# btourn/Neural-Networks-parallel-training-with-MPI

Measured on AMD Instinct MI355X. Metric: samples_per_sec_whole_node, higher is better.
Workload: dtype bf16; 1 GPU; model=mlp_512x4_regression(512-512-512-512-1), global_batch=8192, parallelism=dp1, rows_per_gpu=8192, uneven_split=False, device=cuda, comm=none, graph=True, graph_chunk=128, overlap=True, grouped=True, schedule=rowband, grad_wire_bytes_per_rank=0, n_buckets=3

## Files before the change

neural-networks-parallel-training-with-mpi_amd/csrc/bindings.cpp:

```cpp
#include <pybind11/pybind11.h>
#include <pybind11/stl.h>

#include <stdexcept>
#include <string>

#include "comm/rccl_comm.h"
#include "host/shm_comm.h"
#include "kernels/common.h"
#include "kernels/kernels.h"
#include "knobs.h"

namespace py = pybind11;
using namespace nnmpi;

namespace nnmpi {
void set_sgd_tiles(int v);
}
#if NNMPI_EXPERIMENTS_BUILD
namespace nnmpi {
void set_wgrad_multi_stamps(unsigned long long* buf);
void set_wgm_tile(int t);
}
#endif

// ... 43 lines not shown
  pk.n = (int)py::len(l);
  for (int t = 0; t < pk.n; ++t) {
    auto e = l[t].cast<py::tuple>();
    pk.start[t] = e[0].cast<long long>();
    pk.M[t] = e[1].cast<int>();
    pk.N[t] = e[2].cast<int>();
    pk.pkf[t] = P<bf16>(e[3].cast<uptr>());
    pk.pkd[t] = P<bf16>(e[4].cast<uptr>());
  }
  return true;
}

static void rb_packed_args(const py::object& o, RowbandArgs& a) {
  if (o.is_none()) return;
  auto l = o.cast<py::list>();
  if ((int)py::len(l) != a.nh) throw std::runtime_error("rowband: one (Pf, Pd) pair per hidden layer");
  for (int i = 0; i < a.nh; ++i) {
    auto t = l[i].cast<py::tuple>();
    a.Pf[i] = P<const bf16>(t[0].cast<uptr>());
    a.Pd[i] = P<const bf16>(t[1].cast<uptr>());
  }
}

PYBIND11_MODULE(_nnmpi_hip, m) {
  m.doc() = "MI355X-native kernels and RCCL runtime for nnmpi_amd";

  m.def("arch", []() {
    int dev = 0;
    check(hipGetDevice(&dev), "hipGetDevice");
    hipDeviceProp_t prop;
    check(hipGetDeviceProperties(&prop, dev), "hipGetDeviceProperties");
    return std::string(prop.gcnArchName);
  });
  m.def("cu_count", []() {
    int dev = 0, n = 0;
    check(hipGetDevice(&dev), "hipGetDevice");
    check(hipDeviceGetAttribute(&n, hipDeviceAttributeMultiprocessorCount, dev), "attr");
    return n;
  });
  m.def("source_hash", []() { return std::string(nnmpi_source_hash()); });
  m.def("rccl_version", []() {
    int v = 0;
    ncclGetVersion(&v);
    return v;
  });

  m.def("linear_fwd_bf16", [](uptr X, int ldx, uptr W, int ldw, uptr bias, uptr Y, int ldy, int M,
                              int N, int K, int act, uptr s) {
    check(linear_fwd_bf16(P<const bf16>(X), ldx, P<const bf16>(W), ldw, P<const float>(bias),
                          P<bf16>(Y), ldy, M, N, K, act, S(s)), "linear_fwd_bf16");
  });
  m.def("linear_dgrad_bf16", [](uptr dZ, int lddz, uptr W, int ldw, uptr Ap, int ldap, uptr dX,
                                int lddx, int M, int N, int K, int act, uptr s) {
    check(linear_dgrad_bf16(P<const bf16>(dZ), lddz, P<const bf16>(W), ldw, P<const bf16>(Ap), ldap,
                            P<bf16>(dX), lddx, M, N, K, act, S(s)), "linear_dgrad_bf16");
  });
  m.def("gemm_w4_fwd", [](uptr X, int ldx, uptr W, int ldw, uptr bias, uptr Y, int ldy, int M, int N,
                          int K, int act, uptr s) {
    if (!gemm_w4_fwd) throw std::runtime_error("gemm_w4_fwd: experiments build only (NNMPI_BUILD_EXPERIMENTS=1)");
    check(gemm_w4_fwd(P<const bf16>(X), ldx, P<const bf16>(W), ldw, P<const float>(bias), P<bf16>(Y),
                      ldy, M, N, K, act, S(s)), "gemm_w4_fwd");
  });
  m.def("set_gemm_impl", knob(&set_gemm_impl));
  m.def("get_gemm_impl", &get_gemm_impl);
  m.def("set_gemm_tile", knob(&set_gemm_tile));
  m.def("set_gemm_variant", knob(&set_gemm_variant));
  m.def("set_fwd_variant", knob(&set_fwd_variant));
  m.def("set_store_policy", knob(&set_store_policy));
  m.def("set_slab_store_policy", knob(&set_slab_store_policy));
  m.def("set_pp256_order", knob(&set_pp256_order));
  m.def("set_head_xcd_rows", knob(&set_head_xcd_rows));
  m.def("linear_fwd_bf16_stamped", [](uptr X, int ldx, uptr W, int ldw, uptr bias, uptr Y, int ldy,
                                      int M, int N, int K, uptr st, uptr s) {
#if NNMPI_EXPERIMENTS_BUILD
    check(linear_fwd_bf16_stamped(P<const bf16>(X), ldx, P<const bf16>(W), ldw, P<const float>(bias),
                                  P<bf16>(Y), ldy, M, N, K, P<unsigned long long>(st), S(s)),
          "linear_fwd_bf16_stamped");
#else
    experiments_only("linear_fwd_bf16_stamped");
#endif
  });
  m.def("set_group_async", knob(&set_group_async));
  m.def("set_wgrad_splits", knob(&set_wgrad_splits));
  m.def("wgrad_workspace_bytes", &wgrad_workspace_bytes);
  m.def("wgrad_splits", &wgrad_splits);
  m.def("linear_wgrad_bf16", [](uptr dZ, int lddz, uptr X, int ldx, uptr dW, uptr db, int M, int N,
                                int K, uptr ws, uptr s, py::object sgd) {
    SgdFuse f{};
    const bool fu = to_sgd(sgd, f);
    check(linear_wgrad_bf16(P<const bf16>(dZ), lddz, P<const bf16>(X), ldx, P<float>(dW), P<float>(db),
                            M, N, K, P<float>(ws), S(s), fu ? &f : nullptr), "linear_wgrad_bf16");
  }, py::arg("dZ"), py::arg("lddz"), py::arg("X"), py::arg("ldx"), py::arg("dW"), py::arg("db"),
     py::arg("M"), py::arg("N"), py::arg("K"), py::arg("ws"), py::arg("s"), py::arg("sgd") = py::none());
  m.def("wide_pair_wgrad_ok", &wide_pair_wgrad_ok);
  m.def("wide_pair_dgrad_ok", &wide_pair_dgrad_ok);
  m.def("set_wide_pair", knob(&set_wide_pair));
  m.def("experiments_built", &experiments_built);
  m.def("experiments_on", &experiments_on);
  m.def("cu_hold", [](int blocks, double seconds, uptr s) {
    if (!cu_hold) throw std::runtime_error("cu_hold: experiments build only (NNMPI_BUILD_EXPERIMENTS=1)");
    check(cu_hold(blocks, seconds, S(s)), "cu_hold");
  });
  m.def("set_head_general_valu", knob(&set_head_general_valu));
  m.def("head_general_mfma_ok", &head_general_mfma_ok);
  m.def("set_sgd_epilogue", knob(&set_sgd_epilogue));
  m.def("set_pp_prefetch", knob(&set_pp_prefetch));
  m.def("set_rb_band_map", knob(&set_rb_band_map));
  m.def("cu_mask_stream", [](std::vector<uint32_t> mask) {
    if (!exp_cu_mask_stream)
      throw std::runtime_error("cu_mask_stream: experiments build only (NNMPI_BUILD_EXPERIMENTS=1)");
    hipStream_t st = nullptr;
    check(exp_cu_mask_stream(mask.data(), (int)mask.size(), &st), "cu_mask_stream");
    return reinterpret_cast<uptr>(st);
  });
  m.def("stream_destroy", [](uptr st) { check(hipStreamDestroy(S(st)), "stream_destroy"); });
  m.def("set_stage_epi", knob(&set_stage_epi));
  m.def("wgrad_defer_ok", &wgrad_defer_ok);
  m.def("linear_wgrad_bf16_out16_defer", [](uptr dZ, int lddz, uptr X, int ldx, uptr dW16, uptr db16,
                                            int M, int N, int K, py::object other, uptr g16o, uptr s) {
    SgdFuse f{};
    if (!to_sgd(other, f)) throw std::runtime_error("deferred update needs its SGD operands");
    check(linear_wgrad_bf16_out16_defer(P<const bf16>(dZ), lddz, P<const bf16>(X), ldx, P<bf16>(dW16),
                                        P<bf16>(db16), M, N, K, f, P<const bf16>(g16o), S(s)),
          "linear_wgrad_bf16_out16_defer");
  });
  m.def("wide_pair_wgrad_dgrad_bf16", [](uptr dZ, int lddz, uptr X, int ldx, uptr dW, uptr db, int M,
                                         int N, int K, py::object sgd, uptr dZ2, int lddz2, uptr W2,
                                         int ldw2, uptr Ap2, int ldap2, uptr dX2, int lddx2, int M2,
                                         int N2, int K2, int act2, uptr s) {
    WgradArgs w{P<const bf16>(dZ), lddz, P<const bf16>(X), ldx, P<float>(dW), P<float>(db), M, N, K,
                nullptr, SgdFuse{}};
    to_sgd(sgd, w.sg);
    DgradArgs d{P<const bf16>(dZ2), lddz2, P<const bf16>(W2), ldw2, P<const bf16>(Ap2), ldap2,
                P<bf16>(dX2), lddx2, M2, N2, K2, act2};
    check(wide_pair(w, &d, nullptr, S(s)), "wide_pair_wgrad_dgrad_bf16");
  });
  m.def("wide_pair_wgrad_wgrad_bf16", [](uptr dZ, int lddz, uptr X, int ldx, uptr dW, uptr db, int M,
                                         int N, int K, py::object sgd, uptr dZ2, int lddz2, uptr X2,
                                         int ldx2, uptr dW2, uptr db2, int M2, int N2, int K2,
                                         py::object sgd2, uptr s) {
    WgradArgs w{P<const bf16>(dZ), lddz, P<const bf16>(X), ldx, P<float>(dW), P<float>(db), M, N, K,
                nullptr, SgdFuse{}};
    to_sgd(sgd, w.sg);
    WgradArgs w2{P<const bf16>(dZ2), lddz2, P<const bf16>(X2), ldx2, P<float>(dW2), P<float>(db2), M2,
                 N2, K2, nullptr, SgdFuse{}};
    to_sgd(sgd2, w2.sg);
    check(wide_pair(w, nullptr, &w2, S(s)), "wide_pair_wgrad_wgrad_bf16");
  });
  m.def("linear_wgrad_bf16_out16", [](uptr dZ, int lddz, uptr X, int ldx, uptr dW16, uptr db16,
                                      int M, int N, int K, uptr s) {
    check(linear_wgrad_bf16_ex(P<const bf16>(dZ), lddz, P<const bf16>(X), ldx, nullptr, nullptr,
                               M, N, K, nullptr, S(s),
                               nullptr, nullptr, P<bf16>(dW16), P<bf16>(db16)),
          "linear_wgrad_bf16_out16");
  });
  m.def("gemm_bf16_tile", [](uptr A, int lda, int la, uptr B, int ldb, int lb, int M, int N, int K,
                             uptr C, int ldc, int tile, uptr s) {
    check(gemm_bf16_generic_tile(P<const bf16>(A), lda, la, P<const bf16>(B), ldb, lb, M, N, K,
                                 P<float>(C), ldc, tile, S(s)), "gemm_bf16_tile");
  });
  m.def("gemm_bf16", [](uptr A, int lda, int la, uptr B, int ldb, int lb, int M, int N, int K, uptr C,
                        int ldc, uptr s) {
    check(gemm_bf16_generic(P<const bf16>(A), lda, la, P<const bf16>(B), ldb, lb, M, N, K, P<float>(C),
                            ldc, S(s)), "gemm_bf16");
  });
  m.def("linear_fwd_f32", [](uptr X, int ldx, uptr W, int ldw, uptr bias, uptr Y, int ldy, int M,
// ... 402 lines not shown
```

neural-networks-parallel-training-with-mpi_amd/csrc/kernels/gemm_bf16.hip:

```cpp
#include "gemm_tiles.h"
#include "knobs.h"

namespace nnmpi {

static int g_stage_epi = -1;
void set_stage_epi(int on) { g_stage_epi = on; }
static int stage_epi() {
  if (g_stage_epi < 0) {
    const char* e = knob_env("NNMPI_STAGE_EPI");
    g_stage_epi = (e && e[0] == '1') ? 1 : 0;
  }
  return g_stage_epi;
}
static int g_sgd_serial = -1;
void set_sgd_epilogue(int form) { g_sgd_serial = form; }
static int sgd_serial() {
  if (g_sgd_serial < 0) {
    const char* e = knob_env("NNMPI_SGD_SERIAL");
    g_sgd_serial = (e && e[0] >= '0' && e[0] <= '2') ? e[0] - '0' : 0;
  }
  return g_sgd_serial;
}
static int g_store_pol = 0;

// ... 1020 lines not shown
  int* flag = reinterpret_cast<int*>(smem + 60 * 1024);
  if (tid == 0) {
    const int old = __hip_atomic_fetch_add(cw, 1, __ATOMIC_RELAXED, __HIP_MEMORY_SCOPE_AGENT);
    int mode = 0;
    if (old == S - 1) {
      mode = 2;
    } else {
      int polls = 0;
      while (ld_sc1_i(cw) < S && ++polls < WGM_SPIN) __builtin_amdgcn_s_sleep(8);
      if (polls < WGM_SPIN &&
          __hip_atomic_fetch_add(cw + 1 + split, 1, __ATOMIC_RELAXED, __HIP_MEMORY_SCOPE_AGENT) == 0)
        mode = 1;
    }
    if (mode == 2)
      mode = __hip_atomic_fetch_add(cw + 1 + split, 1, __ATOMIC_RELAXED, __HIP_MEMORY_SCOPE_AGENT) == 0 ? 2 : 3;
    flag[0] = mode;
  }
  __syncthreads();
  const int mode = flag[0];
  __syncthreads();
  if (mode == 0) return;
  if (mode == 1 || mode == 2) wgm_portion(p, f, smem, tx, ty, split);
  if (mode >= 2) {
    for (int o = 1; o < S; ++o) {
      const int pp = (split + o) % S;
      if (tid == 0)
        flag[0] = __hip_atomic_fetch_add(cw + 1 + pp, 1, __ATOMIC_RELAXED, __HIP_MEMORY_SCOPE_AGENT) == 0;
      __syncthreads();
      const int mine = flag[0];
      __syncthreads();
      if (mine) wgm_portion(p, f, smem, tx, ty, pp);
    }
  }
}

template <int GA, int NS, bool ST = false, bool FIX = false>
__global__ void __launch_bounds__(GRP_THREADS, (NS == 0 || GA >= 3 || FIX || ST) ? 2 : 4) wgrad_multi_kernel(WgradMultiParams g) {
  extern __shared__ __attribute__((aligned(1024))) char smem[];
  if constexpr (FIX) {
    if ((int)blockIdx.x >= g.gemm_blocks) {
      slab_reduce_any(g.tail_ws, g.tail, blockIdx.x - g.gemm_blocks, g.tail_nb_main, g.tail_nb_bias,
                      reinterpret_cast<f32x4*>(smem));
      return;
    }
  }
  if constexpr (ST) {
    if (threadIdx.x == 0) {
      g.stamps[blockIdx.x * 4 + 0] = __builtin_amdgcn_s_memrealtime();
      g.stamps[blockIdx.x * 4 + 2] = __builtin_amdgcn_s_getreg(20 | (31 << 11));
      g.stamps[blockIdx.x * 4 + 3] = __builtin_amdgcn_s_getreg(4 | (31 << 11));
    }
  }
  int bid = blockIdx.x;
#pragma unroll
  for (int j = 0; j < RB_MAXL; ++j) {
    if (j >= g.nj) break;
    if (bid < g.blocks[j]) {
      const int l = xcd_remap(bid, g.blocks[j]);
      if (l >= g.n[j]) break;
      const int split = l / g.tiles[j], t = l % g.tiles[j];
      unsigned long long* kst = ST ? g.stamps + 1024 * 4 + (long long)blockIdx.x * 128 : nullptr;
      if constexpr (FIX) {
        constexpr int MI = GRP_BM / GRP_WGM / 16, NJ = GRP_BN / GRP_WGN / 16;
        f32x4 acc[MI * NJ], accb[MI];
        dma_gemm_tile<GRP_BM, GRP_BN, GRP_WGM, GRP_WGN, XMAJ, XMAJ, EPI_F32, ACT_NONE, true, NS, GA, ST,
                      true>(g.wg[j], smem, t % g.gx[j], t / g.gx[j], split, kst, acc, accb);
        wgm_fixup(g.wg[j], g.fix[j], smem, t % g.gx[j], t / g.gx[j], split, t, acc, accb);
      } else if constexpr (NS == 0) {
        wg_reg_tile(g.wg[j], smem, t % g.gx[j], t / g.gx[j], split);
      } else {
        dma_gemm_tile<GRP_BM, GRP_BN, GRP_WGM, GRP_WGN, XMAJ, XMAJ, EPI_F32, ACT_NONE, true, NS, GA, ST>(
            g.wg[j], smem, t % g.gx[j], t / g.gx[j], split, kst);
      }
      break;
    }
    bid -= g.blocks[j];
  }
  if constexpr (ST) {
    __syncthreads();
    if (threadIdx.x == 0) g.stamps[blockIdx.x * 4 + 1] = __builtin_amdgcn_s_memrealtime();
  }
}

#if NNMPI_EXPERIMENTS_BUILD
constexpr int WGH_BM = 128, WGH_BN = 64, WGH_WGM = 2, WGH_WGN = 2;
constexpr int WGH_THREADS = 64 * WGH_WGM * WGH_WGN;
constexpr int WGH_SMEM = 2 * (WGH_BM + WGH_BN) * GEMM_BK * 2;

template <int GA>
__global__ void __launch_bounds__(WGH_THREADS, 2) wgrad_multi_h_kernel(WgradMultiParams g) {
  extern __shared__ __attribute__((aligned(1024))) char smem[];
  int bid = blockIdx.x;
#pragma unroll
  for (int j = 0; j < RB_MAXL; ++j) {
    if (j >= g.nj) break;
    if (bid < g.blocks[j]) {
      const int l = xcd_remap(bid, g.blocks[j]);
      if (l >= g.n[j]) break;
      const int split = l / g.tiles[j], t = l % g.tiles[j];
      dma_gemm_tile<WGH_BM, WGH_BN, WGH_WGM, WGH_WGN, XMAJ, XMAJ, EPI_F32, ACT_NONE, true, 2, GA>(
          g.wg[j], smem, t % g.gx[j], t / g.gx[j], split);
      break;
    }
    bid -= g.blocks[j];
  }
}

static int g_wgm_tile = -1;
void set_wgm_tile(int t) { g_wgm_tile = t; }
static int wgm_tile() {
  if (g_wgm_tile < 0) {
    const char* e = knob_env("NNMPI_WGM_TILE");
    g_wgm_tile = (e && e[0] == '1') ? 1 : 0;
  }
  return g_wgm_tile;
}
#else
static constexpr int wgm_tile() { return 0; }
#endif

template <int GA, int NS>
static void* wgm_fn(bool fix, bool st) {
#if NNMPI_EXPERIMENTS_BUILD
  if (fix) return st ? (void*)wgrad_multi_kernel<GA, NS, true, true> : (void*)wgrad_multi_kernel<GA, NS, false, true>;
  return st ? (void*)wgrad_multi_kernel<GA, NS, true, false> : (void*)wgrad_multi_kernel<GA, NS, false, false>;
#else
  return (fix || st) ? nullptr : (void*)wgrad_multi_kernel<GA, NS, false, false>;
#endif
}

static hipError_t wgm_launch(const WgradMultiParams& g, int nb, bool fix, hipStream_t s) {
  static const int env_ga = [] {
    const char* e = knob_env("NNMPI_WGM_ASYNC");
    return (e && e[0] >= '0' && e[0] <= '4') ? e[0] - '0' : -1;
  }();
  int ga = g_group_async >= 0 ? std::min(g_group_async, 4) : env_ga >= 0 ? env_ga : WGM_ASYNC_DEFAULT;
  int ns = wgm_stages();
  if (fix && ns == 0) ns = 2;
  if (ga < 2) ga = 2;
  const bool st = g.stamps != nullptr;
  void* f = nullptr;
#if NNMPI_EXPERIMENTS_BUILD
  if (ns == 0) f = st ? (void*)wgrad_multi_kernel<2, 0, true> : (void*)wgrad_multi_kernel<2, 0>;
#else
  if (ns == 0) f = st ? nullptr : (void*)wgrad_multi_kernel<2, 0>;
#endif
  else if (ns == 3) f = ga == 2 ? wgm_fn<2, 3>(fix, st) : ga == 3 ? wgm_fn<3, 3>(fix, st) : wgm_fn<4, 3>(fix, st);
  else if (ns == WGM_NS) f = ga == 2 ? wgm_fn<2, WGM_NS>(fix, st) : ga == 3 ? wgm_fn<3, WGM_NS>(fix, st)
                                                                   : wgm_fn<4, WGM_NS>(fix, st);
  else f = ga == 2 ? wgm_fn<2, 2>(fix, st) : ga == 3 ? wgm_fn<3, 2>(fix, st) : wgm_fn<4, 2>(fix, st);
  if (!f) return hipErrorNotSupported;
  const int smem = (ns == 0 ? 2 : ns) * (GRP_BM + GRP_BN) * GEMM_BK * 2;
  static void* attr_done[64] = {};
  bool seen = false;
  for (void*& a : attr_done) {
    if (a == f) { seen = true; break; }
    if (!a) { a = f; break; }
  }
  if (!seen) (void)hipFuncSetAttribute(f, hipFuncAttributeMaxDynamicSharedMemorySize, smem);
  hipLaunchKernelGGL(reinterpret_cast<void (*)(WgradMultiParams)>(f), dim3(nb), dim3(GRP_THREADS), smem, s, g);
  return hipGetLastError();
}

int wgrad_multi_splits(int nj, int M, int N, int K) {
  const int tiles = ((M + GRP_BM - 1) / GRP_BM) * ((N + GRP_BN - 1) / GRP_BN);
  const int ksteps = (K + GEMM_BK - 1) / GEMM_BK;
  int s = std::max(1, 256 / std::max(1, nj * tiles));
  s = std::min(s, std::max(1, ksteps / 4));
  if (g_wgrad_splits > 0 && g_wgrad_splits < s) s = g_wgrad_splits;
  return s;
}

hipError_t wgrad_multi(const WgradArgs* jobs, int nj, const int* splits, SlabReduce* pending,
                       hipStream_t s) {
  if (nj < 1 || nj > RB_MAXL) return hipErrorInvalidValue;
  WgradMultiParams g{};
  g.nj = nj;
  int nb = 0;
  for (int j = 0; j < nj; ++j) {
    const WgradArgs& a = jobs[j];
    if (wgrad_tile(a.M, a.N) != 128 || a.db == nullptr || a.ws == nullptr || a.dW16 != nullptr)
      return hipErrorInvalidValue;
    const int want = (splits && splits[j] > 0) ? splits[j] : wgrad_multi_splits(nj, a.M, a.N, a.K);
    GemmParams p;
    const int sp = make_wgrad_s(a, p, pending[j], want);
    if (sp == 1) {
      p.C = a.ws; p.c_split_stride = (long long)a.M * a.N; p.sg = SgdFuse{};
      p.bias_grad = a.ws + (size_t)a.M * a.N; p.bg_split_stride = a.M;
      p.c16 = nullptr; p.bg16 = nullptr;
      pending[j] = SlabReduce{a.ws, 1, (long long)a.M * a.N, a.M, a.N, a.dW, a.N,
                              a.ws + (size_t)a.M * a.N, a.M, a.db, nullptr, 0, 0.f, nullptr, a.sg};
    }
    set_extents<XMAJ, XMAJ>(p);
    p.store_pol = slab_store_pol();
    g.wg[j] = p;
#if NNMPI_EXPERIMENTS_BUILD
    const int bn = wgm_tile() == 1 ? WGH_BN : GRP_BN;
#else
    const int bn = GRP_BN;
#endif
    g.gx[j] = (p.N + bn - 1) / bn;
    g.tiles[j] = g.gx[j] * ((p.M + GRP_BM - 1) / GRP_BM);
    g.n[j] = g.tiles[j] * sp;
    g.blocks[j] = (g.n[j] + 7) & ~7;
    nb += g.blocks[j];
  }
#if NNMPI_EXPERIMENTS_BUILD
  if (wgm_tile() == 1) {
    static const int env_ga = [] {
      const char* e = knob_env("NNMPI_WGM_ASYNC");
      return (e && e[0] >= '2' && e[0] <= '4') ? e[0] - '0' : -1;
    }();
    const int ga = env_ga == 3 ? 3 : env_ga == 4 ? 4 : 2;
    void* f = ga == 3 ? (void*)wgrad_multi_h_kernel<3> : ga == 4 ? (void*)wgrad_multi_h_kernel<4>
                                                               : (void*)wgrad_multi_h_kernel<2>;
    static void* attr_done[4] = {};
    bool seen = false;
    for (void*& a : attr_done) {
      if (a == f) { seen = true; break; }
      if (!a) { a = f; break; }
    }
    if (!seen) (void)hipFuncSetAttribute(f, hipFuncAttributeMaxDynamicSharedMemorySize, WGH_SMEM);
    hipLaunchKernelGGL(reinterpret_cast<void (*)(WgradMultiParams)>(f), dim3(nb), dim3(WGH_THREADS),
                       WGH_SMEM, s, g);
    return hipGetLastError();
  }
#endif
  g.stamps = g_wgm_stamps;
  return wgm_launch(g, nb, false, s);
}

#if NNMPI_EXPERIMENTS_BUILD
int wgrad_fix_counters(int M, int N) {
  return ((M + GRP_BM - 1) / GRP_BM) * ((N + GRP_BN - 1) / GRP_BN) * WGM_CW;
}
#endif

#if NNMPI_EXPERIMENTS_BUILD
hipError_t wgrad_multi_fix(const WgradArgs* jobs, int nj, const int* splits, const WgOut* fix,
                           const SlabReduce* tail, hipStream_t s) {
  if (nj < 1 || nj > RB_MAXL) return hipErrorInvalidValue;
  WgradMultiParams g{};
  g.nj = nj;
// ... 395 lines not shown
```

neural-networks-parallel-training-with-mpi_amd/csrc/kernels/gemm_tiles.h:

```cpp
#pragma once
#include "common.h"
#include "kernels.h"

#include <algorithm>
#include <cstdlib>

namespace nnmpi {

enum Layout : int { KMAJ = 0, XMAJ = 1 };

constexpr int GEMM_BK = 64;
constexpr int GEMM_THREADS = 256;

struct GemmParams {
  const bf16* A;
  const bf16* B;
  int lda, ldb;
  int M, N, K;
  int k_per_split;
  void* C;
  int ldc;
  long long c_split_stride;
  const float* bias;
  const bf16* aux;
// ... 745 lines not shown
      asm volatile("s_waitcnt lgkmcnt(0)" ::: "memory");
      __builtin_amdgcn_sched_barrier(0);
#pragma unroll
      for (int kk = 0; kk < BK / 32; ++kk) {
#pragma unroll
        for (int i = 0; i < MI; ++i)
#pragma unroll
          for (int j = 0; j < NJ; ++j)
            acc[i][j] = __builtin_amdgcn_mfma_f32_16x16x32_bf16(bfr[j][kk], af[i][kk], acc[i][j], 0, 0, 0);
        if constexpr (BIASGRAD) {
          if (do_bg) {
#pragma unroll
            for (int i = 0; i < MI; ++i)
              accb[i] = __builtin_amdgcn_mfma_f32_16x16x32_bf16(ones, af[i][kk], accb[i], 0, 0, 0);
          }
        }
      }
    } else {
#pragma unroll
      for (int kk = 0; kk < BK / 32; ++kk) {
        bf16x8 af[MI], bfr[NJ];
#pragma unroll
        for (int i = 0; i < MI; ++i) af[i] = read_frag<BM, LA>(cur, wm * WM + i * 16, kk, lane);
#pragma unroll
        for (int j = 0; j < NJ; ++j) bfr[j] = read_frag<BN, LB>(cur + A_BYTES, wn * WN + j * 16, kk, lane);
#pragma unroll
        for (int i = 0; i < MI; ++i)
#pragma unroll
          for (int j = 0; j < NJ; ++j)
            acc[i][j] = __builtin_amdgcn_mfma_f32_16x16x32_bf16(bfr[j], af[i], acc[i][j], 0, 0, 0);
        if constexpr (BIASGRAD) {
          if (do_bg) {
#pragma unroll
            for (int i = 0; i < MI; ++i)
              accb[i] = __builtin_amdgcn_mfma_f32_16x16x32_bf16(ones, af[i], accb[i], 0, 0, 0);
          }
        }
      }
    }
    if constexpr (KST) {
      if (tid == 0 && t < 32) kst[4 * t + 3] = __builtin_amdgcn_s_memtime();
    }
    asm volatile("s_waitcnt lgkmcnt(0)" ::: "memory");
  }
  if constexpr (RET) {
#pragma unroll
    for (int i = 0; i < MI; ++i) {
#pragma unroll
      for (int j = 0; j < NJ; ++j) acc_out[i * NJ + j] = acc[i][j];
      accb_out[i] = accb[i];
    }
    return;
  }
  if constexpr (BM == 128 && BN == 128 && NS * STAGE >= 128 * 128 * 4) {
    if (lepi_ok<EPI>(p)) {
      lds_epilogue<WGM, WGN, EPI, ACT>(p, acc, smem, m0, n0, wm, wn, w, lane, split);
      if constexpr (BIASGRAD) {
        if (do_bg && (lane >> 4) == 0) {
#pragma unroll
          for (int i = 0; i < MI; ++i) {
            const int m = m0 + wm * WM + i * 16 + (lane & 15);
            if (m >= p.M) continue;
            float* g = p.bias_grad + split * p.bg_split_stride + m;
            if (p.sg.g_base) sgd_fused_store(p.sg, g, accb[i][0]);
            else *g = accb[i][0];
          }
        }
      }
      return;
    }
  }
  gemm_epilogue<BM, BN, WGM, WGN, EPI, ACT, BIASGRAD>(p, acc, accb, do_bg, m0, n0, wm, wn, lane, split,
                                                      EPI == EPI_BIAS_ACT ? bias_pre : nullptr);
}

template <int BM, int BN, int WGM, int WGN, int LA, int LB, int EPI, int ACT, bool BIASGRAD, int NS>
__global__ void __launch_bounds__(64 * WGM * WGN) gemm_bf16_dma_kernel(GemmParams p) {
  extern __shared__ __attribute__((aligned(1024))) char smem[];
  const int gx = gridDim.x, gy = gridDim.y;
  const int bid = xcd_remap(blockIdx.y * gx + blockIdx.x, gx * gy);
  dma_gemm_tile<BM, BN, WGM, WGN, LA, LB, EPI, ACT, BIASGRAD, NS>(p, smem, bid % gx, bid / gx, blockIdx.z);
}

constexpr int PP_HALF = 16384;
constexpr int PP_BUF = 4 * PP_HALF;
constexpr int PP_SMEM = 2 * PP_BUF;
constexpr int PP_THREADS = 512;

template <bool OTHER = false>
__device__ __forceinline__ void sgd_epilogue_lds_256(const GemmParams& p, const f32x4 (&acc)[8][4],
                                                     char* smem, int m0, int n0, int wm, int wn,
                                                     int w, int lane, int split) {
  const SgdFuse& f = OTHER ? p.sg2 : p.sg;
  const float lr = f.hp[0], mom = f.hp[1], damp = f.hp[2], wd = f.hp[3], gs = f.hp[4];
  const bool nest = f.nesterov != 0, first = f.first != 0;
  const float* cbase = reinterpret_cast<const float*>(p.C) + split * p.c_split_stride;
  const long long base = OTHER ? 0 : cbase - f.g_base;
  f32x4* img = reinterpret_cast<f32x4*>(smem);
#pragma unroll
  for (int h = 0; h < 2; ++h) {
    __syncthreads();
#pragma unroll
    for (int ii = 0; ii < 4; ++ii) {
      const int r = wm * 64 + ii * 16 + (lane & 15);
#pragma unroll
      for (int j = 0; j < 4; ++j) {
        const int cv = ((j >> 1) * 128 + wn * 32 + (j & 1) * 16) / 4 + (lane >> 4);
        img[r * 64 + (cv ^ (r & 15))] = acc[h * 4 + ii][j];
      }
    }
    __syncthreads();
#pragma unroll
    for (int sb = 0; sb < 2; ++sb) {
      f32x4 pv[8], bv[8];
      f32x4 gov[OTHER ? 8 : 1];
#pragma unroll
      for (int k = 0; k < 8; ++k) {
        const int r = w * 16 + sb * 8 + k;
        const long long o = base + (long long)(m0 + h * 128 + r) * p.ldc + n0 + lane * 4;
        pv[k] = *reinterpret_cast<const f32x4*>(f.p_base + o);
        bv[k] = *reinterpret_cast<const f32x4*>(f.m_base + o);
        if constexpr (OTHER) {
          const bf16x4 gq = *reinterpret_cast<const bf16x4*>(p.g16o + o);
          gov[k] = f32x4{(float)gq[0], (float)gq[1], (float)gq[2], (float)gq[3]};
        }
      }
#pragma unroll
      for (int k = 0; k < 8; ++k) {
        const int r = w * 16 + sb * 8 + k;
        const long long o = base + (long long)(m0 + h * 128 + r) * p.ldc + n0 + lane * 4;
        const f32x4 a = img[r * 64 + (lane ^ (r & 15))];
        f32x4 g = a;
        if constexpr (OTHER) {
          g = gov[k];
          bf16x4 o16;
#pragma unroll
          for (int e = 0; e < 4; ++e) o16[e] = (bf16)a[e];
          *reinterpret_cast<bf16x4*>(p.c16 + (long long)(m0 + h * 128 + r) * p.ldc + n0 + lane * 4) = o16;
        }
        f32x4 q = pv[k], b = bv[k];
#pragma unroll
        for (int e = 0; e < 4; ++e) {
          float bb = b[e];
          q[e] = sgd_elem(q[e], g[e], bb, lr, mom, damp, wd, gs, nest, first);
          b[e] = bb;
        }
        *reinterpret_cast<f32x4*>(f.p_base + o) = q;
        if (mom != 0.f) *reinterpret_cast<f32x4*>(f.m_base + o) = b;
        if (f.s_base) {
          bf16x4 sv;
#pragma unroll
          for (int e = 0; e < 4; ++e) sv[e] = (bf16)q[e];
          *reinterpret_cast<bf16x4*>(f.s_base + o) = sv;
        }
      }
    }
  }
}

template <int ACT>
__device__ __forceinline__ void bias_act_lds_256(const GemmParams& p, const f32x4 (&acc)[8][4],
                                                 char* smem, int m0, int n0, int wm, int wn, int w,
                                                 int lane) {
  bf16x4* img = reinterpret_cast<bf16x4*>(smem);
  f32x4 bias[4];
#pragma unroll
// ... 273 lines not shown
```

neural-networks-parallel-training-with-mpi_amd/csrc/kernels/kernels.h:

```cpp
#pragma once
#include "knobs.h"
#include <hip/hip_runtime.h>
#include <stddef.h>
#include <stdint.h>

namespace nnmpi {

typedef __bf16 bf16;

constexpr int RB_MAXL_PK = 4;

struct SgdFuse {
  const float* g_base;
  float* p_base;
  float* m_base;
  bf16* s_base;
  const float* hp;
  int nesterov;
  int first;
};

struct SlabReduce {
  const float* ws;
  int S;
  long long stride;
  int M, N;
  float* out;
  int ldo;
  const float* bws;
  long long bstride;
  float* bout;
  const float* loss_part;
  int n_loss_part;
  float loss_scale;
  float* loss_out;
  SgdFuse sg;
  int sgd_serial = 0;
  bf16* pkf = nullptr;
  bf16* pkd = nullptr;
};

enum Epi : int { EPI_BIAS_ACT = 0, EPI_DACT = 1, EPI_F32 = 2 };
enum Loss : int { LOSS_MSE = 0, LOSS_XENT = 1 };

hipError_t linear_fwd_bf16(const bf16* X, int ldx, const bf16* W, int ldw, const float* bias,
                           bf16* Y, int ldy, int M, int N, int K, int act, hipStream_t s);
__attribute__((weak)) hipError_t gemm_w4_fwd(const bf16* X, int ldx, const bf16* W, int ldw, const float* bias, bf16* Y,
                       int ldy, int M, int N, int K, int act, hipStream_t s);
hipError_t linear_dgrad_bf16(const bf16* dZ, int lddz, const bf16* W, int ldw, const bf16* Aprev,
                             int lda_prev, bf16* dX, int lddx, int M, int N, int K, int act,
                             hipStream_t s);
int wgrad_splits(int M, int N, int K);
void set_gemm_impl(int impl);
int get_gemm_impl();
void set_gemm_tile(int t);
void set_gemm_variant(int v);
void set_fwd_variant(int v);
void set_pp_prefetch(int v);
void set_pp256_order(int epi, int idx);
void set_store_policy(int p);
void set_slab_store_policy(int p);
void set_head_xcd_rows(int v);
hipError_t linear_fwd_bf16_stamped(const bf16* X, int ldx, const bf16* W, int ldw, const float* bias,
                                   bf16* Y, int ldy, int M, int N, int K, unsigned long long* stamps,
                                   hipStream_t s);
void set_group_async(int m);
void set_wgrad_splits(int s);
size_t wgrad_workspace_bytes(int M, int N, int K);
hipError_t linear_wgrad_bf16(const bf16* dZ, int lddz, const bf16* X, int ldx, float* dW,
                             float* db, int M, int N, int K, float* ws, hipStream_t s,
                             const SgdFuse* sgd = nullptr);
hipError_t gemm_bf16_generic(const bf16* A, int lda, int la, const bf16* B, int ldb, int lb,
                             int M, int N, int K, float* C, int ldc, hipStream_t s);
hipError_t gemm_bf16_generic_tile(const bf16* A, int lda, int la, const bf16* B, int ldb, int lb,
                                  int M, int N, int K, float* C, int ldc, int tile, hipStream_t s);
hipError_t splitk_reduce(const float* ws, int S, long long stride, int M, int N, float* out,
                         int ldo, const float* bws, long long bstride, float* bout,
                         const float* loss_part, int n_loss_part, float loss_scale,
                         float* loss_out, hipStream_t s, const SgdFuse* sgd = nullptr);
hipError_t slab_reduce(const SlabReduce& r, hipStream_t s);
hipError_t linear_wgrad_bf16_ex(const bf16* dZ, int lddz, const bf16* X, int ldx, float* dW,
                                float* db, int M, int N, int K, float* ws, hipStream_t s,
                                const SgdFuse* sgd, SlabReduce* pending, bf16* dW16, bf16* db16);
hipError_t linear_wgrad_bf16_deferred(const bf16* dZ, int lddz, const bf16* X, int ldx, float* dW,
                                      float* db, int M, int N, int K, float* ws, hipStream_t s,
                                      const SgdFuse* sgd, SlabReduce* pending);
struct DgradArgs {
  const bf16* dZ; int lddz; const bf16* W; int ldw; const bf16* Aprev; int lda_prev;
  bf16* dX; int lddx; int M, N, K, act;
};
struct WgradArgs {
  const bf16* dZ; int lddz; const bf16* X; int ldx; float* dW; float* db; int M, N, K;
  float* ws; SgdFuse sg;
  bf16* dW16 = nullptr; bf16* db16 = nullptr;
};
void set_bwd_group(int on);
bool bwd_group_supported(int rows, int out_f, int in_f);
hipError_t bwd_group(const DgradArgs* dg, const WgradArgs* wg, const SlabReduce* red,
                     SlabReduce* wg_pending, hipStream_t s);
bool wide_pair_wgrad_ok(int rows, int out_f, int in_f);
bool wide_pair_dgrad_ok(int rows, int out_f, int in_f);
hipError_t wide_pair(const WgradArgs& w1, const DgradArgs* dg, const WgradArgs* w2, hipStream_t s);
void set_wide_pair(int on);
bool experiments_built();
void set_sgd_epilogue(int form);
void set_stage_epi(int on);
bool wgrad_defer_ok(int M, int N, int K);
hipError_t linear_wgrad_bf16_out16_defer(const bf16* dZ, int lddz, const bf16* X, int ldx, bf16* dW16,
                                         bf16* db16, int M, int N, int K, const SgdFuse& other,
                                         const bf16* g16o, hipStream_t s);

constexpr int RB_MAXL = 4;
struct RowbandArgs {
  const bf16* X; int ldx;
  int rows, H, nh, act;
  int in;
  const bf16* Pf[RB_MAXL];
  const bf16* Pd[RB_MAXL];
  const bf16* W[RB_MAXL];
  const float* b[RB_MAXL];
  bf16* a[RB_MAXL];
  bf16* dz[RB_MAXL];
  const float* wh; const float* bh;
  const float* y;
  float inv_count;
  float* wslab; float* bslab; float* loss_part;
  int band_map;
  unsigned long long* stamps = nullptr;
  int out_pol = 0;
  int* zero_words = nullptr;
  int n_zero = 0;
  int* xsync = nullptr;
  float* hx = nullptr;
  int rbs_bands = 0;
  int rbs_map = 0;
  int rbs_local = 0;
  bf16* ka[RB_MAXL] = {};
  bf16* kz[RB_MAXL] = {};
  int kbands = 0;
};
bool rowband_split_ok(int rows, int H, int in, int nh, int act);
void set_rb_split(int v);
void set_rb_wgsmall(int v);
int rowband_error_word();
int rowband_split_stamp_slots();
void set_rb_store_policy(int pol);
void set_rb_fixup(int on);
void set_rowband_stamps(unsigned long long* buf);
int rowband_stamp_slots();
int rowband_blocks(int rows);
// ... 142 lines not shown
```

neural-networks-parallel-training-with-mpi_amd/utils/knobs.py:

```python
from __future__ import annotations

import os
from typing import Dict, Optional

EXPERIMENTS = "NNMPI_EXPERIMENTS"

KNOBS = {
    "NNMPI_ROWBAND": "row-band step schedule (0 off)",
    "NNMPI_ROWBAND_MIN_ROWS": "smallest batch that takes the row-band step",
    "NNMPI_RB_SPLITS": "row-band weight-gradient split-K slabs",
    "NNMPI_RB_PLAN": "row-band split-K plan (0 one launch, 1 phased; RowbandStep::plan)",
    "NNMPI_DEFER": "deferred bucket updates in weight-gradient epilogues (0 off)",
    "NNMPI_DEFER_WAIT": "deferred update waits per chunk / per layer",
    "NNMPI_CHUNK_MIN_TILES": "tiles per output-row chunk bucket",
    "NNMPI_BF16_REDUCE": "bf16 all-reduce algorithm (acc32 | rccl)",
    "NNMPI_F32_REDUCE": "fp32 all-reduce algorithm (ordered | rccl)",
    "NNMPI_SHM": "shared-memory all-reduce of CPU ranks (0: gloo)",
    "NNMPI_CPU_NATIVE": "native host step of tiny CPU models (0: PyTorch)",
    "NNMPI_STAGE_EPI": "LDS-staged 256x256 forward epilogue",
    "NNMPI_SGD_SERIAL": "SGD epilogue form",
    "NNMPI_PP_PREFETCH": "SGD-operand prefetch in the 256x256 weight gradient",
    "NNMPI_RB_BANDMAP": "XCD-contiguous band order of the row-band kernel",
    "NNMPI_RB_STORE": "row-band copy-out store policy (0 plain, 1 nt, 2 sc1)",
    "NNMPI_RB_SPLIT": "column-split row-band kernel for small batches: 0 off, 2 / 4 / 8 blocks per band, else auto",
    "NNMPI_RB_SPLIT_WAVES": "column-split row-band kernel: waves per block at 4 / 2 blocks per band (4 or 8)",
    "NNMPI_RB_WGSMALL": "small-batch row-band weight gradients: 1 un-split tiles with the update fused, 0 split-K slabs",
    "NNMPI_WGS_ASYNC": "small-batch weight-gradient LDS read mode (2 / 3 / 4, dma_gemm_tile ASYNC_TR)",
    "NNMPI_WGS_STAGES": "small-batch weight-gradient DMA ring stages (2 / 3 / 4 / 6 / 8)",
    "NNMPI_RB_FIXUP": "row-band split-K combine inside the weight-gradient launch (0: own launch)",
    "NNMPI_GEMM": "GEMM main loop (1 register-staged, 2 LDS-DMA)",
    "NNMPI_SLAB_STORE": "split-K slab store policy",
    "NNMPI_GROUP": "grouped backward launch (0 off)",
    "NNMPI_GRAPH_UPLOAD": "hipGraphUpload after instantiation (0 off)",
    "NNMPI_PAIR": "wide backward pair launches (experiments build)",
    "NNMPI_COMM_STANDIN": "k:gbps -- k CUs held after every bucket collective (standin.hip)",
    "NNMPI_WG_STAGES": "grouped weight-gradient launch DMA ring stages (default 2; 4)",
    "NNMPI_WG_REG": "register-staged operands in the grouped weight-gradient launch (A/B)",
    "NNMPI_WGM_ASYNC": "LDS read mode of the row-band weight-gradient launch (2; 3 pipelined)",
    "NNMPI_WGM_TILE": "row-band weight-gradient tile (0: 128x128, 8 waves; 1: 128x64, 4 waves)",
    "NNMPI_HEAD_BLOCKS": "block cap of the fused multi-output head (default 256)",
    "NNMPI_HEAD_FUSED": "multi-output head + weight gradient in one kernel (0: two launches)",
}

INTERNAL = {"NNMPI_SUPERVISED", "NNMPI_ATTEMPT", "NNMPI_PROGRESS_FILE", "NNMPI_RESULT_FILE",
            "NNMPI_LAUNCHER", "NNMPI_RDZV_KEY"}


def experiments() -> bool:
    return os.environ.get(EXPERIMENTS) == "1"


def knob(name: str, default: Optional[str] = None) -> Optional[str]:
    assert name in KNOBS, name
    if not experiments():
        return default
    return os.environ.get(name, default)


def seen() -> Dict[str, dict]:
    on = experiments()
    out = {}
    for k, v in sorted(os.environ.items()):
        if not k.startswith("NNMPI_") or k in INTERNAL:
            continue
        out[k] = {"value": v, "honoured": (on if k in KNOBS else True)}
    return out
```

Before: 115.2 million samples/s.

## Add warp-specialized loader waves feeding the row-band weight-gradient DMA ring

Adds a weight-gradient tile kernel in which extra loader waves issue the DMA loads into a 3-stage LDS ring while the eight compute waves only read fragments and run MFMAs. It is enabled by default for the row-band weight-gradient launch when no fixup is used, and the default LDS read mode becomes the pipelined one. The aim is to take global-to-LDS load issue and waiting off the compute waves so memory and matrix work overlap better. In exchange each block carries extra threads and a deeper ring of shared memory, which can lower occupancy, and the barrier-based handoff between loader and compute waves has to stay balanced.

```diff
diff --git a/neural-networks-parallel-training-with-mpi_amd/csrc/bindings.cpp b/neural-networks-parallel-training-with-mpi_amd/csrc/bindings.cpp
--- a/neural-networks-parallel-training-with-mpi_amd/csrc/bindings.cpp
+++ b/neural-networks-parallel-training-with-mpi_amd/csrc/bindings.cpp
@@ -149,6 +149,7 @@
   });
   m.def("set_group_async", knob(&set_group_async));
   m.def("set_wgrad_splits", knob(&set_wgrad_splits));
+  m.def("set_wgm_loader", knob(&set_wgm_loader));
   m.def("wgrad_workspace_bytes", &wgrad_workspace_bytes);
   m.def("wgrad_splits", &wgrad_splits);
   m.def("linear_wgrad_bf16", [](uptr dZ, int lddz, uptr X, int ldx, uptr dW, uptr db, int M, int N,
diff --git a/neural-networks-parallel-training-with-mpi_amd/csrc/kernels/gemm_bf16.hip b/neural-networks-parallel-training-with-mpi_amd/csrc/kernels/gemm_bf16.hip
--- a/neural-networks-parallel-training-with-mpi_amd/csrc/kernels/gemm_bf16.hip
+++ b/neural-networks-parallel-training-with-mpi_amd/csrc/kernels/gemm_bf16.hip
@@ -1126,6 +1126,72 @@
   }
 }
 
+constexpr int WGL_NS = 3, WGL_L = 4;
+constexpr int WGL_ASYNC_DEFAULT = 3;
+template <int GA, int NS, int L, bool ST = false>
+__global__ void __launch_bounds__(GRP_THREADS + 64 * L) wgrad_multi_ld_kernel(WgradMultiParams g) {
+  extern __shared__ __attribute__((aligned(1024))) char smem[];
+  if constexpr (ST) {
+    if (threadIdx.x == 0) {
+      g.stamps[blockIdx.x * 4 + 0] = __builtin_amdgcn_s_memrealtime();
+      g.stamps[blockIdx.x * 4 + 2] = __builtin_amdgcn_s_getreg(20 | (31 << 11));
+      g.stamps[blockIdx.x * 4 + 3] = __builtin_amdgcn_s_getreg(4 | (31 << 11));
+    }
+  }
+  int bid = blockIdx.x;
+#pragma unroll
+  for (int j = 0; j < RB_MAXL; ++j) {
+    if (j >= g.nj) break;
+    if (bid < g.blocks[j]) {
+      const int l = xcd_remap(bid, g.blocks[j]);
+      if (l >= g.n[j]) break;
+      const int split = l / g.tiles[j], t = l % g.tiles[j];
+      unsigned long long* kst = ST ? g.stamps + 1024 * 4 + (long long)blockIdx.x * 128 : nullptr;
+      wgrad_loader_tile<NS, L, GA, ST>(g.wg[j], smem, t % g.gx[j], t / g.gx[j], split, kst);
+      break;
+    }
+    bid -= g.blocks[j];
+  }
+  if constexpr (ST) {
+    __syncthreads();
+    if (threadIdx.x == 0) g.stamps[blockIdx.x * 4 + 1] = __builtin_amdgcn_s_memrealtime();
+  }
+}
+
+constexpr int WGM_LOADER_DEFAULT = 1;
+static int g_wgm_loader = -1;
+void set_wgm_loader(int v) { g_wgm_loader = v; }
+static int wgm_loader() {
+  if (g_wgm_loader < 0) {
+    const char* e = knob_env("NNMPI_WGM_LOADER");
+    g_wgm_loader = (e && e[0] >= '0' && e[0] <= '9') ? std::atoi(e) : WGM_LOADER_DEFAULT;
+  }
+  return g_wgm_loader;
+}
+
+template <int NS, int L>
+static void* wgl_fn(int ga, bool st) {
+#if NNMPI_EXPERIMENTS_BUILD
+  if (st) return ga >= 3 ? (void*)wgrad_multi_ld_kernel<3, NS, L, true> : (void*)wgrad_multi_ld_kernel<2, NS, L, true>;
+#else
+  if (st) return nullptr;
+#endif
+  return ga >= 3 ? (void*)wgrad_multi_ld_kernel<3, NS, L> : (void*)wgrad_multi_ld_kernel<2, NS, L>;
+}
+
+static void* wgl_select(int form, int ga, bool st, int& ns, int& l) {
+  ns = WGL_NS; l = WGL_L;
+  if (form == 1 || form == 10 * WGL_NS + WGL_L) return wgl_fn<WGL_NS, WGL_L>(ga, st);
+#if NNMPI_EXPERIMENTS_BUILD
+  ns = form / 10; l = form % 10;
+  if (form == 32) return wgl_fn<3, 2>(ga, st);
+  if (form == 34) return wgl_fn<3, 4>(ga, st);
+  if (form == 42) return wgl_fn<4, 2>(ga, st);
+  if (form == 44) return wgl_fn<4, 4>(ga, st);
+#endif
+  return nullptr;
+}
+
 #if NNMPI_EXPERIMENTS_BUILD
 constexpr int WGH_BM = 128, WGH_BN = 64, WGH_WGM = 2, WGH_WGN = 2;
 constexpr int WGH_THREADS = 64 * WGH_WGM * WGH_WGN;
@@ -1178,23 +1244,32 @@
     const char* e = knob_env("NNMPI_WGM_ASYNC");
     return (e && e[0] >= '0' && e[0] <= '4') ? e[0] - '0' : -1;
   }();
-  int ga = g_group_async >= 0 ? std::min(g_group_async, 4) : env_ga >= 0 ? env_ga : WGM_ASYNC_DEFAULT;
   int ns = wgm_stages();
   if (fix && ns == 0) ns = 2;
+  const int loader = (fix || ns == 0) ? 0 : wgm_loader();
+  int ga = g_group_async >= 0 ? std::min(g_group_async, 4) : env_ga >= 0 ? env_ga
+           : loader != 0 ? WGL_ASYNC_DEFAULT : WGM_ASYNC_DEFAULT;
   if (ga < 2) ga = 2;
   const bool st = g.stamps != nullptr;
   void* f = nullptr;
+  int smem = (ns == 0 ? 2 : ns) * (GRP_BM + GRP_BN) * GEMM_BK * 2, threads = GRP_THREADS;
+  if (loader != 0) {
+    int lns = 0, ll = 0;
+    f = wgl_select(loader, ga, st, lns, ll);
+    smem = lns * (GRP_BM + GRP_BN) * GEMM_BK * 2;
+    threads = GRP_THREADS + 64 * ll;
+  } else if (ns == 0) {
 #if NNMPI_EXPERIMENTS_BUILD
-  if (ns == 0) f = st ? (void*)wgrad_multi_kernel<2, 0, true> : (void*)wgrad_multi_kernel<2, 0>;
+    f = st ? (void*)wgrad_multi_kernel<2, 0, true> : (void*)wgrad_multi_kernel<2, 0>;
 #else
-  if (ns == 0) f = st ? nullptr : (void*)wgrad_multi_kernel<2, 0>;
+    f = st ? nullptr : (void*)wgrad_multi_kernel<2, 0>;
 #endif
+  }
   else if (ns == 3) f = ga == 2 ? wgm_fn<2, 3>(fix, st) : ga == 3 ? wgm_fn<3, 3>(fix, st) : wgm_fn<4, 3>(fix, st);
   else if (ns == WGM_NS) f = ga == 2 ? wgm_fn<2, WGM_NS>(fix, st) : ga == 3 ? wgm_fn<3, WGM_NS>(fix, st)
                                                                    : wgm_fn<4, WGM_NS>(fix, st);
   else f = ga == 2 ? wgm_fn<2, 2>(fix, st) : ga == 3 ? wgm_fn<3, 2>(fix, st) : wgm_fn<4, 2>(fix, st);
   if (!f) return hipErrorNotSupported;
-  const int smem = (ns == 0 ? 2 : ns) * (GRP_BM + GRP_BN) * GEMM_BK * 2;
   static void* attr_done[64] = {};
   bool seen = false;
   for (void*& a : attr_done) {
@@ -1202,7 +1277,7 @@
     if (!a) { a = f; break; }
   }
   if (!seen) (void)hipFuncSetAttribute(f, hipFuncAttributeMaxDynamicSharedMemorySize, smem);
-  hipLaunchKernelGGL(reinterpret_cast<void (*)(WgradMultiParams)>(f), dim3(nb), dim3(GRP_THREADS), smem, s, g);
+  hipLaunchKernelGGL(reinterpret_cast<void (*)(WgradMultiParams)>(f), dim3(nb), dim3(threads), smem, s, g);
   return hipGetLastError();
 }
 
diff --git a/neural-networks-parallel-training-with-mpi_amd/csrc/kernels/gemm_tiles.h b/neural-networks-parallel-training-with-mpi_amd/csrc/kernels/gemm_tiles.h
--- a/neural-networks-parallel-training-with-mpi_amd/csrc/kernels/gemm_tiles.h
+++ b/neural-networks-parallel-training-with-mpi_amd/csrc/kernels/gemm_tiles.h
@@ -851,6 +851,163 @@
   dma_gemm_tile<BM, BN, WGM, WGN, LA, LB, EPI, ACT, BIASGRAD, NS>(p, smem, bid % gx, bid / gx, blockIdx.z);
 }
 
+__device__ __forceinline__ void wgl_bias_store(const GemmParams& p, int m, int split, float v) {
+  if (m >= p.M) return;
+  if (p.bg16) { p.bg16[m] = (bf16)v; return; }
+  float* g = p.bias_grad + split * p.bg_split_stride + m;
+  if (p.sg.g_base) sgd_fused_store(p.sg, g, v);
+  else *g = v;
+}
+
+template <int NS, int L, int GA = 2, bool KST = false>
+__device__ __forceinline__ void wgrad_loader_tile(const GemmParams& p, char* smem, int tx, int ty,
+                                                  int split, unsigned long long* kst = nullptr) {
+  constexpr int BM = 128, BN = 128, WGM = 2, WGN = 4, NC = WGM * WGN, BK = GEMM_BK;
+  constexpr int A_BYTES = BM * BK * 2, B_BYTES = BN * BK * 2, STAGE = A_BYTES + B_BYTES;
+  constexpr int WM = BM / WGM, WN = BN / WGN, MI = WM / 16, NJ = WN / 16;
+  static_assert(NS >= 3 && NS * STAGE >= 128 * 128 * 4, "ring holds the epilogue's fp32 image");
+  static_assert(GA == 2 || GA == 3, "LDS read mode");
+
+  const int tid = threadIdx.x, lane = tid & 63;
+  const int w = __builtin_amdgcn_readfirstlane(tid >> 6);
+  const int m0 = ty * BM, n0 = tx * BN;
+  const int kbeg = split * p.k_per_split;
+  const int kend = min(p.K, kbeg + p.k_per_split);
+  const int nt = kend > kbeg ? (kend - kbeg + BK - 1) / BK : 0;
+  const bool lepi = lepi_ok<EPI_F32>(p);
+
+  if (w >= NC) {
+    const int lw = w - NC;
+    using PlanA = DmaPlan<BM, XMAJ, L>;
+    using PlanB = DmaPlan<BN, XMAJ, L>;
+    constexpr int PER_STAGE = PlanA::NI + PlanB::NI;
+    static_assert((NS - 2) * PER_STAGE <= 63, "vmcnt counts at most 63");
+    const __amdgpu_buffer_rsrc_t rsA = __builtin_amdgcn_make_buffer_rsrc((void*)p.A, (short)0, (int)p.a_bytes, 0x00020000);
+    const __amdgpu_buffer_rsrc_t rsB = __builtin_amdgcn_make_buffer_rsrc((void*)p.B, (short)0, (int)p.b_bytes, 0x00020000);
+    PlanA da;
+    PlanB db;
+    da.init(lw, lane, m0, p.M, p.lda);
+    db.init(lw, lane, n0, p.N, p.ldb);
+#pragma unroll
+    for (int t = 0; t < NS - 1; ++t) {
+      if (t < nt) {
+        char* st = smem + t * STAGE;
+        da.issue(rsA, st, lw, kbeg + t * BK, kend);
+        db.issue(rsB, st + A_BYTES, lw, kbeg + t * BK, kend);
+      }
+    }
+    unsigned long long issued = 0;
+    for (int t = 0; t < nt; ++t) {
+      const int newer = min(NS - 2, nt - 1 - t);
+      if (NS >= 4 && newer >= 2) wait_vm<2 * PER_STAGE>();
+      else if (newer >= 1) wait_vm<PER_STAGE>();
+      else wait_vm<0>();
+      __builtin_amdgcn_s_barrier();
+      if constexpr (KST) {
+        if (lw == 0 && lane == 0 && t >= 1 && t <= 32) kst[4 * (t - 1) + 2] = issued;
+      }
+      if (t + NS - 1 < nt) {
+        char* st = smem + ((t + NS - 1) % NS) * STAGE;
+        da.issue(rsA, st, lw, kbeg + (t + NS - 1) * BK, kend);
+        db.issue(rsB, st + A_BYTES, lw, kbeg + (t + NS - 1) * BK, kend);
+      }
+      if constexpr (KST) issued = __builtin_amdgcn_s_memtime();
+    }
+    if constexpr (KST) {
+      if (lw == 0 && lane == 0 && nt >= 1 && nt <= 32) kst[4 * (nt - 1) + 2] = issued;
+    }
+    if (lepi) {
+      __builtin_amdgcn_s_barrier();
+      __builtin_amdgcn_s_barrier();
+    }
+    return;
+  }
+
+  const int wm = w / WGN, wn = w % WGN;
+  f32x4 acc[MI][NJ];
+#pragma unroll
+  for (int i = 0; i < MI; ++i)
+#pragma unroll
+    for (int j = 0; j < NJ; ++j) acc[i][j] = f32x4{0.f, 0.f, 0.f, 0.f};
+  f32x4 accb = f32x4{0.f, 0.f, 0.f, 0.f};
+  const bool do_bg = tx == 0;
+  bf16x8 ones;
+#pragma unroll
+  for (int e = 0; e < 8; ++e) ones[e] = (bf16)1.0f;
+
+  for (int t = 0; t < nt; ++t) {
+    if constexpr (KST) {
+      if (tid == 0 && t < 32) kst[4 * t] = __builtin_amdgcn_s_memtime();
+    }
+    __builtin_amdgcn_s_barrier();
+    if constexpr (KST) {
+      if (tid == 0 && t < 32) kst[4 * t + 1] = __builtin_amdgcn_s_memtime();
+    }
+    const char* cur = smem + (t % NS) * STAGE;
+    if constexpr (GA == 3) {
+      constexpr int NR = 2 * (MI + NJ);
+      static_assert(NR <= 15, "lgkmcnt counts at most 15 outstanding LDS reads");
+      bf16x8 af[2][MI], bfr[2][NJ];
+#pragma unroll
+      for (int kk = 0; kk < 2; ++kk) {
+#pragma unroll
+        for (int i = 0; i < MI; ++i) af[kk][i] = read_frag_async<BM, XMAJ>(cur, wm * WM + i * 16, kk, lane);
+#pragma unroll
+        for (int j = 0; j < NJ; ++j) bfr[kk][j] = read_frag_async<BN, XMAJ>(cur + A_BYTES, wn * WN + j * 16, kk, lane);
+      }
+#pragma unroll
+      for (int kk = 0; kk < 2; ++kk) {
+        if (kk == 0) asm volatile("s_waitcnt lgkmcnt(%0)" ::"n"(NR) : "memory");
+        else asm volatile("s_waitcnt lgkmcnt(0)" ::: "memory");
+#pragma unroll
+        for (int i = 0; i < MI; ++i) asm volatile("" : "+v"(af[kk][i]));
+#pragma unroll
+        for (int j = 0; j < NJ; ++j) asm volatile("" : "+v"(bfr[kk][j]));
+        __builtin_amdgcn_sched_barrier(0);
+#pragma unroll
+        for (int i = 0; i < MI; ++i) {
+#pragma unroll
+          for (int j = 0; j < NJ; ++j)
+            acc[i][j] = __builtin_amdgcn_mfma_f32_16x16x32_bf16(bfr[kk][j], af[kk][i], acc[i][j], 0, 0, 0);
+          if (do_bg && wn == i) accb = __builtin_amdgcn_mfma_f32_16x16x32_bf16(ones, af[kk][i], accb, 0, 0, 0);
+        }
+        __builtin_amdgcn_sched_barrier(0);
+      }
+    } else {
+#pragma unroll
+      for (int kk = 0; kk < BK / 32; ++kk) {
+        bf16x8 af[MI], bfr[NJ];
+#pragma unroll
+        for (int i = 0; i < MI; ++i) af[i] = read_frag_async<BM, XMAJ>(cur, wm * WM + i * 16, kk, lane);
+#pragma unroll
+        for (int j = 0; j < NJ; ++j) bfr[j] = read_frag_async<BN, XMAJ>(cur + A_BYTES, wn * WN + j * 16, kk, lane);
+        asm volatile("s_waitcnt lgkmcnt(0)" ::: "memory");
+        __builtin_amdgcn_sched_barrier(0);
+#pragma unroll
+        for (int i = 0; i < MI; ++i) {
+#pragma unroll
+          for (int j = 0; j < NJ; ++j)
+            acc[i][j] = __builtin_amdgcn_mfma_f32_16x16x32_bf16(bfr[j], af[i], acc[i][j], 0, 0, 0);
+          if (do_bg && wn == i) accb = __builtin_amdgcn_mfma_f32_16x16x32_bf16(ones, af[i], accb, 0, 0, 0);
+        }
+      }
+    }
+    if constexpr (KST) {
+      if (tid == 0 && t < 32) kst[4 * t + 3] = __builtin_amdgcn_s_memtime();
+    }
+    asm volatile("s_waitcnt lgkmcnt(0)" ::: "memory");
+  }
+  if (lepi) {
+    lds_epilogue<WGM, WGN, EPI_F32, ACT_NONE>(p, acc, smem, m0, n0, wm, wn, w, lane, split);
+  } else {
+    f32x4 nob[MI];
+#pragma unroll
+    for (int i = 0; i < MI; ++i) nob[i] = f32x4{0.f, 0.f, 0.f, 0.f};
+    gemm_epilogue<BM, BN, WGM, WGN, EPI_F32, ACT_NONE, false>(p, acc, nob, false, m0, n0, wm, wn, lane, split);
+  }
+  if (do_bg && (lane >> 4) == 0) wgl_bias_store(p, m0 + wm * WM + wn * 16 + (lane & 15), split, accb[0]);
+}
+
 constexpr int PP_HALF = 16384;
 constexpr int PP_BUF = 4 * PP_HALF;
 constexpr int PP_SMEM = 2 * PP_BUF;
diff --git a/neural-networks-parallel-training-with-mpi_amd/csrc/kernels/kernels.h b/neural-networks-parallel-training-with-mpi_amd/csrc/kernels/kernels.h
--- a/neural-networks-parallel-training-with-mpi_amd/csrc/kernels/kernels.h
+++ b/neural-networks-parallel-training-with-mpi_amd/csrc/kernels/kernels.h
@@ -66,6 +66,7 @@
                                    hipStream_t s);
 void set_group_async(int m);
 void set_wgrad_splits(int s);
+void set_wgm_loader(int v);
 size_t wgrad_workspace_bytes(int M, int N, int K);
 hipError_t linear_wgrad_bf16(const bf16* dZ, int lddz, const bf16* X, int ldx, float* dW,
                              float* db, int M, int N, int K, float* ws, hipStream_t s,
diff --git a/neural-networks-parallel-training-with-mpi_amd/utils/knobs.py b/neural-networks-parallel-training-with-mpi_amd/utils/knobs.py
--- a/neural-networks-parallel-training-with-mpi_amd/utils/knobs.py
+++ b/neural-networks-parallel-training-with-mpi_amd/utils/knobs.py
@@ -37,6 +37,7 @@
     "NNMPI_WG_STAGES": "grouped weight-gradient launch DMA ring stages (default 2; 4)",
     "NNMPI_WG_REG": "register-staged operands in the grouped weight-gradient launch (A/B)",
     "NNMPI_WGM_ASYNC": "LDS read mode of the row-band weight-gradient launch (2; 3 pipelined)",
+    "NNMPI_WGM_LOADER": "row-band weight-gradient tile (1: loader waves fill the DMA ring; 0: the compute waves do)",
     "NNMPI_WGM_TILE": "row-band weight-gradient tile (0: 128x128, 8 waves; 1: 128x64, 4 waves)",
     "NNMPI_HEAD_BLOCKS": "block cap of the fused multi-output head (default 256)",
     "NNMPI_HEAD_FUSED": "multi-output head + weight gradient in one kernel (0: two launches)",
```

Result: no change. 116.1 million samples/s, median of 6 (+0.7%).
